# shuklaayush/halo2-plonky2-verifier

Measured on AMD Instinct MI355X. Metric: FRI-verifier witness cells/sec, higher is better.
Workload: dtype u64

## Files before the change

halo2-plonky2-verifier_amd/csrc/coop.h:

```cpp
#pragma once
#include <type_traits>
#include "valbackend.h"
#include "bntab.h"
#include "glptab.h"

namespace h2w {

constexpr int GLP_RECS_FULL = 12 + 48 + 1 + 12 * 14;
constexpr int GLP_RECS_PARTIAL_ROUND = 4 + 1 + 1 + 11 + 1 + 11;
constexpr int GLP_RECS_PARTIAL = 12 + 1 + 121 + N_PARTIAL_ROUNDS * GLP_RECS_PARTIAL_ROUND;
constexpr int GLP_CONST_WORDS = 360 + 12 + 12 + 12 + 22 + 121 + 242 + 242;
constexpr int GLP_RECS = 2 * HALF_N_FULL_ROUNDS * GLP_RECS_FULL + GLP_RECS_PARTIAL;

__device__ __forceinline__ void wave_sync() { asm volatile("s_waitcnt lgkmcnt(0)" ::: "memory"); __builtin_amdgcn_wave_barrier(); }

__shared__ uint64_t s_glp_k[GLP_CONST_WORDS];
__shared__ uint64_t s_glp_a[SPONGE_WIDTH], s_glp_b[SPONGE_WIDTH];
__shared__ uint64_t s_glp_in[CH_BUF];
__shared__ uint64_t s_glp_m[SPONGE_WIDTH * SPONGE_WIDTH];
__shared__ uint64_t s_glp_x[GLP_AUX_WORDS];
typedef __attribute__((address_space(3))) uint64_t lds64_t;
constexpr int KO_ARC = 0, KO_CIRC = 360, KO_DIAG = 372, KO_FIRST = 384, KO_PRC = 396, KO_INIT = 418, KO_WHAT = 539, KO_VS = 781;
static_assert(KO_VS + 242 == GLP_CONST_WORDS, "Goldilocks constant block layout");
template <bool AUX = false> __device__ __forceinline__ void stage_glp_consts(const h2w_poseidon_consts_t *k, int tid, int nthreads) {
    const uint64_t *src = reinterpret_cast<const uint64_t *>(k);
    for (int i = tid; i < GLP_CONST_WORDS; i += nthreads) s_glp_k[i] = g_load_u64(src + i);
    if constexpr (AUX) { const uint64_t *ax = reinterpret_cast<const uint64_t *>(k + 1); for (int i = tid; i < GLP_AUX_WORDS; i += nthreads) s_glp_x[i] = g_load_u64(ax + i); }
    for (int i = tid; i < SPONGE_WIDTH * SPONGE_WIDTH; i += nthreads) {
        const int r = i / SPONGE_WIDTH, j = i % SPONGE_WIDTH; int d = j - r; if (d < 0) d += SPONGE_WIDTH;
        const uint64_t c = g_load_u64(src + KO_CIRC + d);
        s_glp_m[i] = j == r ? gl_reduce128((u128)c + g_load_u64(src + KO_DIAG + r)) : c;
    }
    __syncthreads();
}
inline bool glp_small_mds(const h2w_poseidon_consts_t &k) {
    for (int i = 0; i < SPONGE_WIDTH; i++) if (k.mds_circ[i] >= (1ull << 26) || k.mds_diag[i] >= (1ull << 26)) return false;
    return true;
}

__device__ __forceinline__ uint64_t gl_add_c(uint64_t x, uint64_t y) {
    uint64_t t = x + y;
    if (t < x || t >= GL_P) t -= GL_P;
    return t;
}
__device__ __forceinline__ uint64_t shfl_up64(uint64_t v, int d) { return __shfl_up(v, d, 64); }

__device__ __forceinline__ uint64_t readlane64(uint64_t v, int src) {
    const unsigned lo = (unsigned)__builtin_amdgcn_readlane((int)(unsigned)v, src), hi = (unsigned)__builtin_amdgcn_readlane((int)(unsigned)(v >> 32), src);
    return ((uint64_t)hi << 32) | lo;
}
template <int N> __device__ __forceinline__ uint64_t row_shr64(uint64_t v) {
    const unsigned lo = (unsigned)__builtin_amdgcn_update_dpp(0, (int)(unsigned)v, 0x110 + N, 0xf, 0xf, true);
    const unsigned hi = (unsigned)__builtin_amdgcn_update_dpp(0, (int)(unsigned)(v >> 32), 0x110 + N, 0xf, 0xf, true);
    return ((uint64_t)hi << 32) | lo;
}
}
#include "glperm.h"
namespace h2w {
constexpr int GLP_LIST_WORDS = 1 + SPONGE_WIDTH;

template <bool COLS, bool VALPH = false, int HASH_MODE = -1> struct CoopSinkT : SinkBase {
    static constexpr bool kCoop = true, kDevSponge = VALPH; static constexpr int kHashMode = HASH_MODE;
    rec_t *recs; uint64_t nrec; fr_t *out; uint64_t cell_off; const uint16_t *ncells; int lane; ColPolicy<COLS> cc;
    lds64_t *lk = nullptr, *la = nullptr, *lb = nullptr, *lm = nullptr, *lx = nullptr;
    uint64_t *glp = nullptr; uint32_t glp_slot = 0; bool small_mds = false;
    __device__ __forceinline__ void bind_lds() { lk = (lds64_t *)s_glp_k; la = (lds64_t *)s_glp_a; lb = (lds64_t *)s_glp_b; lm = (lds64_t *)s_glp_m; if constexpr (VALPH) lx = (lds64_t *)s_glp_x; }
    bool emit = true;
    __device__ __forceinline__ void rec(int t, uint64_t a, uint64_t b, uint64_t c, uint64_t d) {
        if (lane == 0 && emit) g_store_rec(recs + nrec, a, b, c, d);
        nrec++; cell_off += ncells[t];
    }
    __device__ __forceinline__ void cell(const fr_t &v) { if (lane == 0 && emit) g_store_fr(out + cc.map(cell_off), v); cell_off++; }
    __device__ __forceinline__ void skip(uint64_t nr, uint64_t nc) { nrec += nr; cell_off += nc; }
    __device__ __forceinline__ bool coop_load_proof(const ValCfg &cfg) { nrec += cfg.load_nrec; cell_off += cfg.load_ncell; return true; }
    uint64_t sx = 0; int sp_in = 0, sp_out = 0; lds64_t *lin = nullptr;
    __device__ __forceinline__ void sponge_init() { sx = 0; sp_in = sp_out = 0; lin = (lds64_t *)s_glp_in; }
    __device__ __forceinline__ bool sponge_observe(uint64_t t) { sp_out = 0; if (sp_in >= CH_BUF) return false; lin[sp_in++] = t; return true; }
    template <class WordFn> __device__ __forceinline__ bool sponge_observe_words(const uint64_t *proof, int n, WordFn word) {
        sp_out = 0; if (sp_in + n > CH_BUF) return false;
        for (int base = 0; base < n; base += 64) { const int i = base + lane; if (i < n) lin[sp_in + i] = g_load_u64(proof + word(i)); }
        sp_in += n; return true;
    }
    template <class WordFn> __device__ __forceinline__ void stage_words(const uint64_t *proof, int at, int n, WordFn word) {
        for (int base = 0; base < n; base += 64) { const int i = base + lane; if (i < n) lin[at + i] = g_load_u64(proof + word(i)); }
    }
    __device__ __forceinline__ uint64_t staged_word(int i) const { return lin[i]; }
    __device__ __forceinline__ bool sponge_observe_cap(const uint64_t *proof, uint64_t w0, int n, int mode, int L) {
        const int per = mode == 0 ? 4 : 5;
        sp_out = 0; if (sp_in + per * n > CH_BUF) return false;
        for (int base = 0; base < n; base += 64) {
            const int j = base + lane;
            if (j < n) {
                fr_t x; for (int i = 0; i < 4; i++) x.l[i] = g_load_u64(proof + w0 + 4ull * j + i);
                if (mode == 0) for (int i = 0; i < 4; i++) lin[sp_in + 4 * j + i] = x.l[i];
                else for (int t = 0; t < 5; t++) lin[sp_in + 5 * j + t] = fr_bits(x, 56 * t, 56);
            }
        }
        sp_in += per * n;
        if (mode == 1) { const int nl = (56 + L - 1) / L, rem = 56 % L; cell_off += (uint64_t)n * (13 + 5ull * ((nl > 1 ? 1 + 3 * (nl - 1) : 0) + (rem ? 4 : 0))); }
        return true;
    }
    __device__ __forceinline__ void sponge_permute() {
        const uint64_t up = row_shr64<1>(sx), w = lane == 0 ? nrec : up;
        uint64_t *at = emit && lane < GLP_LIST_WORDS ? glp + (uint64_t)glp_slot * GLP_LIST_WORDS + lane : nullptr;
        glp_slot++;
        sx = glp_permute_lanes(sx, lk, lm, lx, lane, small_mds, at, w);
        nrec += GLP_RECS;
        cell_off += perm_cell_count();
    }
    uint64_t perm_cells_ = 0;
    __device__ __forceinline__ uint64_t perm_cell_count() {
        if (perm_cells_ == 0) {
            const uint64_t nG = ncells[T_GLOP], nKA = ncells[T_KA_GLOP];
            perm_cells_ = 2 * HALF_N_FULL_ROUNDS * (12 * nKA + 48 * nG + 12 + 12 * (1 + 13 * nKA)) + 12 * nKA + 12 + 121 * nKA + (uint64_t)N_PARTIAL_ROUNDS * (4 * nG + nKA + nKA + 11 * nKA + 12 + 11 * nKA);
        }
        return perm_cells_;
    }
    __device__ __forceinline__ uint64_t sponge_challenge() {
        if (sp_in) {
            for (int off = 0; off < sp_in; off += SPONGE_RATE) {
                const int len = sp_in - off < SPONGE_RATE ? sp_in - off : SPONGE_RATE;
                if ((lane & 15) < len) sx = lin[off + (lane & 15)];
                sponge_permute();
            }
            sp_in = 0; sp_out = SPONGE_RATE;
        } else if (sp_out == 0) { sponge_permute(); sp_out = SPONGE_RATE; }
        return readlane64(sx, --sp_out);
    }

#if defined(H2W_FLATTEN_CHIPS)
    __device__ __forceinline__
#else
    __device__ __noinline__
#endif
    void coop_poseidon_permute(uint64_t *st, const h2w_poseidon_consts_t *) {
        if constexpr (VALPH) {
            uint64_t w = nrec, x = 0;
#pragma unroll
            for (int i = 0; i < SPONGE_WIDTH; i++) { if (lane == i + 1) w = st[i]; if ((lane & 15) == i) x = st[i]; }
            uint64_t *at = emit && lane < GLP_LIST_WORDS ? glp + (uint64_t)glp_slot * GLP_LIST_WORDS + lane : nullptr;
            glp_slot++;
            x = glp_permute_lanes(x, lk, lm, lx, lane, small_mds, at, w);
#pragma unroll
            for (int i = 0; i < SPONGE_WIDTH; i++) st[i] = readlane64(x, i);
            nrec += GLP_RECS;
            cell_off += perm_cell_count();
            return;
        }
        lds64_t *const K = lk, *const s_a = la, *const s_b = lb;
        rec_t *R = recs + nrec;
        const int l = lane, grp13 = lane / 13, idx13 = lane % 13;
        const bool em = emit;
        auto W = [&](int idx, uint64_t A, uint64_t B, uint64_t C) { if (em) g_store_rec(R + idx, A, B, C, 0); };
        if (l < SPONGE_WIDTH) s_a[l] = st[l];
        wave_sync();
        int base = 0, round_ctr = 0;
        auto full_round = [&]() {
            if (l < SPONGE_WIDTH) {
                uint64_t x = s_a[l]; const uint64_t rc = K[KO_ARC + l + SPONGE_WIDTH * round_ctr];
                W(base + l, rc, 1, x); x = gl_add(x, rc);
                const int sb = base + 12 + 4 * l;
                const uint64_t x2 = gl_mul(x, x); W(sb, x, x, 0);
                const uint64_t x4 = gl_mul(x2, x2); W(sb + 1, x2, x2, 0);
                const uint64_t x6 = gl_mul(x4, x2); W(sb + 2, x4, x2, 0);
                const uint64_t x7 = gl_mul(x6, x); W(sb + 3, x6, x, 0);
                s_b[l] = x7;
            }
            wave_sync();
            const int mb = base + 60;
            if (l == 0) W(mb, 0, 0, 0);
            uint64_t rowres = 0;
#pragma unroll
            for (int pass = 0; pass < 3; pass++) {
                const int rr = pass * 4 + grp13;
                uint64_t c = 0, v = 0, x = 0;
                if (l < 52) {
                    if (idx13 < 12) { c = K[KO_CIRC + idx13]; int vi = idx13 + rr; if (vi >= 12) vi -= 12; v = s_b[vi]; }
                    else { c = K[KO_DIAG + rr]; v = s_b[rr]; }
                    x = gl_mul(c, v);
                }
#pragma unroll
                for (int d = 1; d < 16; d <<= 1) { const uint64_t y = shfl_up64(x, d); if (idx13 >= d) x = gl_add_c(x, y); }
                uint64_t prev = shfl_up64(x, 1); if (idx13 == 0) prev = 0;
                if (l < 52) {
                    const int rb = mb + 1 + 14 * rr;
                    if (idx13 == 0) W(rb, 0, 0, 0);
                    W(rb + 1 + idx13, c, v, prev);
                    if (idx13 == 12) rowres = x;
                }
                if (l < 52 && idx13 == 12) s_a[rr] = rowres;
            }
            wave_sync();
            base += GLP_RECS_FULL; round_ctr++;
        };
        for (int i = 0; i < HALF_N_FULL_ROUNDS; i++) full_round();
        if (l < SPONGE_WIDTH) {
            const uint64_t x = s_a[l], c = K[KO_FIRST + l];
            W(base + l, c, 1, x); s_b[l] = gl_add(x, c);
        }
        wave_sync();
        base += 12;
        if (l == 0) { W(base, 0, 0, 0); s_a[0] = s_b[0]; }
        else if (l < SPONGE_WIDTH) {
            uint64_t res = 0;
            for (int r = 1; r < SPONGE_WIDTH; r++) {
                const uint64_t t = K[KO_INIT + (r - 1) * 11 + (l - 1)], v = s_b[r];
                W(base + 1 + (r - 1) * 11 + (l - 1), t, v, res); res = gl_muladd(t, v, res);
            }
            s_a[l] = res;
        }
        wave_sync();
        base += 122;
        for (int r = 0; r < N_PARTIAL_ROUNDS; r++) {
            if (l == 0) {
                const uint64_t x = s_a[0];
                const uint64_t x2 = gl_mul(x, x); W(base, x, x, 0);
                const uint64_t x4 = gl_mul(x2, x2); W(base + 1, x2, x2, 0);
                const uint64_t x6 = gl_mul(x4, x2); W(base + 2, x4, x2, 0);
                const uint64_t x7 = gl_mul(x6, x); W(base + 3, x6, x, 0);
                const uint64_t c = K[KO_PRC + r];
                W(base + 4, c, 1, x7); s_a[0] = gl_add(x7, c);
            }
            wave_sync();
            const uint64_t s0 = s_a[0];
            {
                uint64_t t = 0, v = 0, x = 0;
                if (l == 0) { t = K[KO_CIRC] + K[KO_DIAG]; v = s0; }
                else if (l < SPONGE_WIDTH) { t = K[KO_WHAT + r * 11 + (l - 1)]; v = s_a[l]; }
                if (l < SPONGE_WIDTH) x = gl_mul(t, v);
#pragma unroll
                for (int d = 1; d < 16; d <<= 1) { const uint64_t y = shfl_up64(x, d); if (l >= d) x = gl_add_c(x, y); }
                uint64_t prev = shfl_up64(x, 1); if (l == 0) prev = 0;
                if (l < SPONGE_WIDTH) W(base + 5 + l, t, v, prev);
                if (l == 0) W(base + 17, 0, 0, 0);
                if (l == SPONGE_WIDTH - 1) s_b[0] = x;
                if (l > 0 && l < SPONGE_WIDTH) {
                    const uint64_t tv = K[KO_VS + r * 11 + (l - 1)];
                    W(base + 17 + l, tv, s0, v); s_b[l] = gl_muladd(tv, s0, v);
                }
            }
            wave_sync();
            if (l < SPONGE_WIDTH) s_a[l] = s_b[l];
            wave_sync();
            base += GLP_RECS_PARTIAL_ROUND;
        }
        round_ctr += N_PARTIAL_ROUNDS;
        for (int i = 0; i < HALF_N_FULL_ROUNDS; i++) full_round();
        for (int i = 0; i < SPONGE_WIDTH; i++) st[i] = s_a[i];
        wave_sync();
        const uint64_t nG = ncells[T_GLOP], nKA = ncells[T_KA_GLOP];
        const uint64_t full_cells = 12 * nKA + 48 * nG + 12 + 12 * (1 + 13 * nKA);
        const uint64_t part_cells = 12 * nKA + 12 + 121 * nKA + (uint64_t)N_PARTIAL_ROUNDS * (4 * nG + nKA + nKA + 11 * nKA + 12 + 11 * nKA);
        nrec += GLP_RECS; cell_off += 2 * HALF_N_FULL_ROUNDS * full_cells + part_cells;
    }
};

#ifndef H2W_QUAD_BLOCK
#define H2W_QUAD_BLOCK 256
#endif
constexpr int QUAD_BLOCK = H2W_QUAD_BLOCK;
constexpr int QUAD_WAVES = QUAD_BLOCK / 64;
struct __attribute__((aligned(16))) sq16_t { unsigned long long x, y; };
__shared__ sq16_t s_bn_tab[BK_X * 2];
__shared__ sq16_t s_bn_val[QUAD_WAVES * BN_NSLOT * BN_SLOT_SQ];
__device__ __forceinline__ void stage_bn_consts(const fr_t *tab, int tid, int nthreads) {
    const sq16_t *src = reinterpret_cast<const sq16_t *>(tab);
    for (int i = tid; i < BK_X * 2; i += nthreads) { sq16_t v; v.x = H2W_GLOAD64(&src[i].x); v.y = H2W_GLOAD64(&src[i].y); s_bn_tab[i] = v; }
    __syncthreads();
}
__device__ __forceinline__ fr_t bnk(int which, int idx) {
    const sq16_t a = s_bn_tab[(which * BK_T + idx) * 2], b = s_bn_tab[(which * BK_T + idx) * 2 + 1];
    fr_t r; r.l[0] = a.x; r.l[1] = a.y; r.l[2] = b.x; r.l[3] = b.y; return r;
}
__device__ __forceinline__ fr_t bnkc(int r) {
    const sq16_t a = s_bn_tab[(BK_XC + r) * 2], b = s_bn_tab[(BK_XC + r) * 2 + 1];
    fr_t v; v.l[0] = a.x; v.l[1] = a.y; v.l[2] = b.x; v.l[3] = b.y; return v;
}
__shared__ uint32_t s_bn_tab9[BK9_N * BK9_W];
__device__ __forceinline__ void stage_bn_consts9(const uint32_t *tab9, int tid, int nthreads) {
    const sq16_t *src = reinterpret_cast<const sq16_t *>(tab9); sq16_t *dst = reinterpret_cast<sq16_t *>(s_bn_tab9);
    for (int i = tid; i < BK9_N * BK9_W / 4; i += nthreads) { sq16_t v; v.x = H2W_GLOAD64(&src[i].x); v.y = H2W_GLOAD64(&src[i].y); dst[i] = v; }
    __syncthreads();
}
__device__ __forceinline__ fr9_t bnk9(int idx) {
    const uint4 a = *reinterpret_cast<const uint4 *>(s_bn_tab9 + idx * BK9_W), b = *reinterpret_cast<const uint4 *>(s_bn_tab9 + idx * BK9_W + 4);
    fr9_t v; v.t[0] = a.x; v.t[1] = a.y; v.t[2] = a.z; v.t[3] = a.w; v.t[4] = b.x; v.t[5] = b.y; v.t[6] = b.z; v.t[7] = b.w; v.t[8] = s_bn_tab9[idx * BK9_W + 8];
    return v;
}
template <int CTRL> __device__ __forceinline__ fr_t quad_dpp(const fr_t &v) {
    fr_t r;
#pragma unroll
    for (int i = 0; i < 4; i++) {
        const unsigned lo = (unsigned)v.l[i], hi = (unsigned)(v.l[i] >> 32);
        const unsigned rlo = (unsigned)__builtin_amdgcn_update_dpp(0, (int)lo, CTRL, 0xf, 0xf, false);
        const unsigned rhi = (unsigned)__builtin_amdgcn_update_dpp(0, (int)hi, CTRL, 0xf, 0xf, false);
        r.l[i] = ((unsigned long long)rhi << 32) | rlo;
    }
    return r;
}
template <int J> __device__ __forceinline__ fr_t quad_bcast(const fr_t &v) { return quad_dpp<J * 0x55>(v); }
__device__ __forceinline__ fr_t quad_up1(const fr_t &v) { return quad_dpp<0x90>(v); }
__device__ __forceinline__ fr_t quad_up2(const fr_t &v) { return quad_dpp<0x44>(v); }

template <int CTRL> __device__ __forceinline__ fr9_t quad_dpp9(const fr9_t &v) {
    fr9_t r;
#pragma unroll
    for (int i = 0; i < 9; i++) r.t[i] = (uint32_t)__builtin_amdgcn_update_dpp(0, (int)v.t[i], CTRL, 0xf, 0xf, false);
    return r;
}
template <int J> __device__ __forceinline__ fr9_t quad_bcast9(const fr9_t &v) { return quad_dpp9<J * 0x55>(v); }
__device__ __forceinline__ fr9_t fr9_sel(bool c, const fr9_t &a, const fr9_t &b) {
    fr9_t r;
#pragma unroll
    for (int i = 0; i < 9; i++) r.t[i] = c ? a.t[i] : b.t[i];
    return r;
}
__device__ __forceinline__ fr9_t fr9_add_if(bool c, const fr9_t &a, const fr9_t &b) {
    fr9_t r;
#pragma unroll
    for (int i = 0; i < 9; i++) r.t[i] = a.t[i] + (c ? b.t[i] : 0u);
    return r;
}
__device__ __forceinline__ fr_t fr_sel(bool c, const fr_t &a, const fr_t &b) {
    fr_t r;
#pragma unroll
    for (int i = 0; i < 4; i++) r.l[i] = c ? a.l[i] : b.l[i];
    return r;
}
struct BnSrc { int kind, idx; };
constexpr BnSrc bV(int s) { return BnSrc{0, s}; }
constexpr BnSrc bK(int i) { return BnSrc{1, i}; }
constexpr BnSrc bA(int o) { return BnSrc{2, o}; }
constexpr BnSrc bB(int o) { return BnSrc{3, o}; }
constexpr BnSrc bn_map_exp5(int c) {
    const int l = c / 12, i = c % 12;
    return (i == 0 || i == 4 || i == 8) ? bK(BK_ZERO) : (i == 1 || i == 2 || i == 10) ? bV(l) : (i == 3 || i == 5 || i == 6) ? bV(4 + l) : (i == 7 || i == 9) ? bV(8 + l) : bV(12 + l);
}
constexpr BnSrc bn_map_ark(int c) {
    const int l = c / 5, i = c % 5;
    return (i == 0 || i == 2) ? bA(l) : i == 1 ? bV(l) : i == 3 ? bK(BK_ONE) : bV(4 + l);
}
constexpr BnSrc bn_map_mix(int c) {
    const int l = c / 16, j = (c % 16) / 4, i = c % 4;
    return i == 0 ? (j == 0 ? bK(BK_ZERO) : bV(4 + 4 * l + j - 1)) : i == 1 ? bA(4 * j + l) : i == 2 ? bV(j) : bV(4 + 4 * l + j);
}
constexpr BnSrc bn_map_consts(int c) { return bA(c); }
constexpr BnSrc bn_map_zero(int) { return bK(BK_ZERO); }
constexpr BnSrc bn_map_partial(int c) {
    if (c < 12) return (c == 0 || c == 4 || c == 8) ? bK(BK_ZERO) : (c == 1 || c == 2 || c == 10) ? bV(0) : (c == 3 || c == 5 || c == 6) ? bV(4) : (c == 7 || c == 9) ? bV(5) : bV(6);
    if (c < 17) return (c == 12 || c == 14) ? bB(0) : c == 13 ? bV(6) : c == 15 ? bK(BK_ONE) : bV(7);
    if (c < 37) { const int j = (c - 17) / 5, i = (c - 17) % 5; return (i == 0 || i == 2) ? bA(j) : i == 1 ? (j == 0 ? bK(BK_ZERO) : bV(8 + j - 1)) : i == 3 ? (j == 0 ? bV(7) : bV(j)) : bV(8 + j); }
    const int k = 1 + (c - 37) / 5, i = (c - 37) % 5;
    return (i == 0 || i == 2) ? bA(4 + k - 1) : i == 1 ? bV(k) : i == 3 ? bV(7) : bV(12 + k - 1);
}

enum { QUAD_VALUES = 1, QUAD_EMIT = 2, QUAD_FUSED = 3 };
constexpr int QUAD_VERDICT = 4;
template <bool COLS, int MODE> struct QuadSinkT : SinkBase {
    static constexpr bool kBnUnits = true; static constexpr int kHashMode = 1;
    rec_t *recs; uint64_t nrec; fr_t *out; uint64_t cell_off; const uint16_t *ncells; int l4; ColPolicy<COLS> cc;
    fr_t *ustate;
    fr_t *sbx;
    int unit_local = 0;
    int my_w = 0, last_w = 0;
    bool act = true;
    __device__ __forceinline__ void set_window(int w, int n_units) { my_w = w; last_w = n_units > 0 ? n_units - 1 : 0; unit_local = 0; act = w == 0; }
    __device__ __forceinline__ void rec(int t, uint64_t a, uint64_t b, uint64_t c, uint64_t d) {
        if (MODE != QUAD_VALUES && l4 == 0 && act) g_store_rec(recs + nrec, a, b, c, d);
        nrec++; cell_off += ncells[t];
    }
    __device__ __forceinline__ void cell(const fr_t &v) { if (MODE != QUAD_VALUES && l4 == 0 && act) g_store_fr(out + cc.map(cell_off), v); cell_off++; }
    __device__ __forceinline__ void skip(uint64_t nr, uint64_t nc) { nrec += nr; cell_off += nc; }
    struct Em {
        sq16_t *val;
        const sq16_t *tabh;
        unsigned long long gdst;
        uint64_t cell0;
        int l;
        ColPolicy<COLS> cc;
    };
    static __device__ __forceinline__ void put(const Em &e, int slot, const fr_t &v) {
        sq16_t *q = e.val + slot * BN_SLOT_SQ; q[0] = sq16_t{v.l[0], v.l[1]}; q[1] = sq16_t{v.l[2], v.l[3]};
    }
    static __device__ __forceinline__ void put_if(const Em &e, bool on, int slot, const fr_t &v) { if (on) put(e, slot, v); }
    template <class MapFn> static __device__ __forceinline__ const sq16_t *src_ptr(const Em &e, MapFn map, int c, const sq16_t *baseA, const sq16_t *baseB) {
        const BnSrc s = map(c);
        return s.kind == 0 ? e.val + s.idx * BN_SLOT_SQ + (e.l & 1) : s.kind == 1 ? e.tabh + s.idx * 2 : s.kind == 2 ? baseA + s.idx * 2 : baseB + s.idx * 2;
    }
    template <int N, class MapFn> __device__ __forceinline__ void flush_layer(Em &e, MapFn map, const sq16_t *baseA, const sq16_t *baseB) {
        constexpr int NP = (N + 1) / 2;
        const bool hiq = e.l >= 2;
        if constexpr (COLS) {
            if (e.cc.hi - e.cell0 < (uint64_t)N || e.cell0 < e.cc.lo) { e = flush_layer_cols<N>(e, map, baseA, baseB); return; }
        }
#pragma unroll
        for (int k0 = 0; k0 < NP; k0 += 4) {
            sq16_t t[4];
#pragma unroll
            for (int u = 0; u < 4; u++) {
                const int k = k0 + u;
                if (k < NP) {
                    const sq16_t *pa = src_ptr(e, map, 2 * k, baseA, baseB), *pb = (2 * k + 1 < N) ? src_ptr(e, map, 2 * k + 1, baseA, baseB) : pa;
                    t[u] = *(hiq ? pb : pa);
                }
            }
#pragma unroll
            for (int u = 0; u < 4; u++) {
                const int k = k0 + u;
                if (k < NP) {
                    unsigned long long *g = reinterpret_cast<unsigned long long *>(e.gdst + (unsigned long long)k * 64);
                    if (2 * k + 1 < N || !hiq) { H2W_GSTORE64(g, t[u].x); H2W_GSTORE64(g + 1, t[u].y); }
                }
            }
        }
        e.cell0 += (uint64_t)N; e.gdst += (unsigned long long)N * 32;
    }
    template <int K0, int K1, int N, class MapFn> static __device__ __forceinline__ void part_load(const Em &e, MapFn map, const sq16_t *baseA, const sq16_t *baseB, sq16_t *t) {
        const bool hiq = e.l >= 2;
#pragma unroll
        for (int k = K0; k < K1; k++) {
            const sq16_t *pa = src_ptr(e, map, 2 * k, baseA, baseB), *pb = (2 * k + 1 < N) ? src_ptr(e, map, 2 * k + 1, baseA, baseB) : pa;
            t[k - K0] = *(hiq ? pb : pa);
        }
    }
    template <int K0, int K1, int N> static __device__ __forceinline__ void part_store(const Em &e, const sq16_t *t) {
        const bool hiq = e.l >= 2;
#pragma unroll
        for (int k = K0; k < K1; k++) {
            unsigned long long *g = reinterpret_cast<unsigned long long *>(e.gdst + (unsigned long long)k * 64);
            if (2 * k + 1 < N || !hiq) { H2W_GSTORE64(g, t[k - K0].x); H2W_GSTORE64(g + 1, t[k - K0].y); }
        }
    }
    typedef __attribute__((address_space(3))) const sq16_t lds_sq16;
    struct Wide { int off0, off1, kind0, kind1; bool has1; int lane; unsigned long long gq; };
    static __device__ __forceinline__ void wide_desc(int pc, int &off, int &kind) {
        const int c = pc >> 1; const BnSrc sd = bn_map_partial(c < 52 ? c : 51);
        kind = sd.kind; off = (sd.kind == 0 ? sd.idx * BN_SLOT_SQ : sd.idx * 2) + (pc & 1);
    }
    static __device__ __forceinline__ Wide wide_init(const Em &e) {
        Wide w; w.lane = threadIdx.x & 63; w.has1 = w.lane < 2 * 52 - 64;
        wide_desc(w.lane, w.off0, w.kind0); wide_desc(w.has1 ? 64 + w.lane : 0, w.off1, w.kind1);
        w.gq = e.gdst - (unsigned long long)e.l * 16;
        return w;
    }
    template <int Q0, int Q1> static __device__ __forceinline__ void wide_load(const Wide &w, lds_sq16 *valw, lds_sq16 *tab, lds_sq16 *baseA, lds_sq16 *baseB, sq16_t *t0, sq16_t *t1) {
        lds_sq16 *b0 = (w.kind0 == 0 ? valw : w.kind0 == 1 ? tab : w.kind0 == 2 ? baseA : baseB) + w.off0;
        lds_sq16 *b1 = (w.kind1 == 0 ? valw : w.kind1 == 1 ? tab : w.kind1 == 2 ? baseA : baseB) + w.off1;
        const int q0 = w.kind0 == 0 ? 2 : 0, q1 = w.kind1 == 0 ? 2 : 0;
#pragma unroll
        for (int q = Q0; q < Q1; q++) { t0[q - Q0].x = b0[q * q0].x; t0[q - Q0].y = b0[q * q0].y; t1[q - Q0].x = b1[q * q1].x; t1[q - Q0].y = b1[q * q1].y; }
    }
    template <int Q0, int Q1> static __device__ __forceinline__ void wide_store(const Wide &w, const sq16_t *t0, const sq16_t *t1) {
#pragma unroll
        for (int q = Q0; q < Q1; q++) {
            const unsigned long long gb = readlane64(w.gq, 4 * q) + (unsigned long long)w.lane * 16;
            unsigned long long *g = reinterpret_cast<unsigned long long *>(gb);
            H2W_GSTORE64(g, t0[q - Q0].x); H2W_GSTORE64(g + 1, t0[q - Q0].y);
            if (w.has1) { H2W_GSTORE64(g + 128, t1[q - Q0].x); H2W_GSTORE64(g + 129, t1[q - Q0].y); }
        }
    }
    template <int N, class MapFn> __device__ __noinline__ Em flush_layer_cols(Em e, MapFn map, const sq16_t *baseA, const sq16_t *baseB) {
        if constexpr (COLS) {
            const bool hiq = e.l >= 2;
            for (int k = 0; k < (N + 1) / 2; k++) {
                const int c = 2 * k + (hiq ? 1 : 0);
                if (c < N) {
                    const sq16_t *pa = src_ptr_rt(e, map, 2 * k, baseA, baseB), *pb = (2 * k + 1 < N) ? src_ptr_rt(e, map, 2 * k + 1, baseA, baseB) : pa;
                    const sq16_t t = *(hiq ? pb : pa);
                    const uint64_t a = e.cc.map(e.cell0 + (uint64_t)c);
                    unsigned long long *g = reinterpret_cast<unsigned long long *>(reinterpret_cast<unsigned long long>(out + a) + (unsigned long long)(e.l & 1) * 16);
                    H2W_GSTORE64(g, t.x); H2W_GSTORE64(g + 1, t.y);
                }
            }
            e.cell0 += (uint64_t)N;
            e.gdst = reinterpret_cast<unsigned long long>(out + e.cc.map(e.cell0)) + (unsigned long long)e.l * 16;
        }
        return e;
    }
    template <class MapFn> static __device__ __forceinline__ const sq16_t *src_ptr_rt(const Em &e, MapFn map, int c, const sq16_t *baseA, const sq16_t *baseB) {
        const BnSrc s = map(c);
        return s.kind == 0 ? e.val + s.idx * BN_SLOT_SQ + (e.l & 1) : s.kind == 1 ? e.tabh + s.idx * 2 : s.kind == 2 ? baseA + s.idx * 2 : baseB + s.idx * 2;
    }
    __device__ __forceinline__ bool level_skip(fr_t &node, bool &zc_ref) {
        if constexpr (MODE != QUAD_EMIT) return false;
        else {
            const int k = unit_local;
            if (k == my_w) return false;
            if (k + 1 == my_w) node = g_load_fr(ustate + (uint64_t)k * 4);
            if (!zc_ref) { cell_off += 1; zc_ref = true; }
            cell_off += 2 * 8 + 4 + BN_PERM_CELLS;
            unit_local = k + 1;
            const int cur = unit_local < last_w ? unit_local : last_w;
            act = cur == my_w;
            return true;
        }
    }
    __device__ __forceinline__ bool tail_skip() const { return MODE == QUAD_VALUES || (MODE == QUAD_EMIT && !act); }
    __device__ __forceinline__ bool bn_emit_inline(fr_t *st, const ValCfg &cfg, bool &zc_ref) {
        if constexpr (MODE == QUAD_VALUES || MODE == QUAD_VERDICT) { bn_values(st, cfg); unit_local++; return true; }
        else if constexpr (MODE == QUAD_FUSED) { bn_emit_cells<false>(st, cfg, zc_ref); return true; }
        else {
            const int k = unit_local++;
            if (k == my_w) bn_emit_cells<true>(st, cfg, zc_ref);
            else {
                if (k + 1 == my_w) {
                    const fr_t *u = ustate + (uint64_t)k * 4;
#pragma unroll
                    for (int i = 0; i < 4; i++) st[i] = g_load_fr(u + i);
                }
                if (!zc_ref) { cell_off += 1; zc_ref = true; }
                cell_off += BN_PERM_CELLS;
            }
            const int cur = unit_local < last_w ? unit_local : last_w;
            act = cur == my_w;
            return true;
        }
    }
    __device__ __noinline__ void bn_values(fr_t *st, const ValCfg &cfg) {
        const int l = l4, lm = l > 0 ? l - 1 : 0; const uint32_t ninv = (uint32_t)cfg.P.ninv & ((1u << 29) - 1);
        fr_t *const sbu = sbx + (uint64_t)unit_local * (BN_PARTIAL_ROUNDS * 3);
        fr9_t S = fr9_mont(fr9_from(fr_sel(l < 2, fr_sel(l == 0, st[0], st[1]), fr_sel(l == 2, st[2], st[3]))), fr9_from(cfg.P.r2), ninv);
        auto sbox = [&]() { const fr9_t X2 = fr9_mont(S, S, ninv), X4 = fr9_mont(X2, X2, ninv); S = fr9_mont(X4, S, ninv); };
        auto mix = [&](int mb) {
            const fr9_t s0 = quad_bcast9<0>(S), s1 = quad_bcast9<1>(S), s2 = quad_bcast9<2>(S), s3 = quad_bcast9<3>(S);
            fr9_t acc = fr9_mont(s0, bnk9(mb + l), ninv);
            acc = fr9_add(fr9_mont(s1, bnk9(mb + 4 + l), ninv), acc);
            acc = fr9_add(fr9_mont(s2, bnk9(mb + 8 + l), ninv), acc);
            S = fr9_norm(fr9_add(fr9_mont(s3, bnk9(mb + 12 + l), ninv), acc));
        };
        S = fr9_norm(fr9_add(S, bnk9(BK_C + l)));
#pragma unroll 1
        for (int half = 0; half < 2; half++) {
            if (half == 1) {
                fr9_t s0p; for (int i = 0; i < 9; i++) s0p.t[i] = 0;
                struct RoundK { fr9_t kp, k2, k1, kc, kx; };
                auto round_k = [&](int r) {
                    const int ix = BK_S + (BN_WIDTH * 2 - 1) * r, ic = BK_C + (BN_FULL_ROUNDS / 2 + 1) * BN_WIDTH + r;
                    RoundK k; k.kp = bnk9(ix - (BN_WIDTH * 2 - 1) + BN_WIDTH + lm);
                    k.k2 = bnk9(ix + (l == 1 ? 0 : l)); k.k1 = bnk9(ix + 1); k.kc = bnk9(ic); k.kx = bnk9(BK9_X + r);
                    return k;
                };
                RoundK kc_ = round_k(0);
#pragma unroll 2
                for (int r = 0; r < BN_PARTIAL_ROUNDS; r++) {
                    const RoundK kn = round_k(r + 1 < BN_PARTIAL_ROUNDS ? r + 1 : r);
                    fr_t *const sb = sbu + (uint64_t)r * 3;
                    const fr9_t s0b = quad_bcast9<0>(S);
                    const fr9_t A_ = fr9_mont(fr9_sel(l == 0, S, s0p), fr9_sel(l == 0, S, kc_.kp), ninv);
                    if constexpr (MODE != QUAD_VERDICT) { if (l == 0) g_store_fr(sb, fr9_pack(A_)); }
                    const fr9_t X2b = quad_bcast9<0>(A_);
                    S = fr9_add_if(l > 0, S, A_);
                    const fr9_t B_ = fr9_mont(fr9_sel(l == 0, X2b, fr9_sel(l == 1, s0b, S)), fr9_sel(l == 0, X2b, kc_.k2), ninv);
                    if constexpr (MODE != QUAD_VERDICT) { if (l == 0) g_store_fr(sb + 1, fr9_pack(B_)); }
                    const fr9_t X4b = quad_bcast9<0>(B_), XAb = quad_bcast9<1>(B_);
                    const fr9_t C_ = fr9_mont(fr9_sel(l == 1, S, X4b), fr9_sel(l == 0, XAb, fr9_sel(l == 1, kc_.k1, s0b)), ninv);
                    if constexpr (MODE != QUAD_VERDICT) { if (l == 2) g_store_fr(sb + 2, fr9_pack(C_)); }
                    s0p = fr9_add(quad_bcast9<2>(C_), kc_.kc);
                    fr9_t incl = fr9_add_if(l == 0, fr9_sel(l < 2, C_, B_), kc_.kx);
                    incl = fr9_add(incl, quad_dpp9<0xB1>(incl));
                    incl = fr9_add(incl, quad_dpp9<0x4E>(incl));
                    S = fr9_norm(fr9_sel(l == 0, incl, S));
                    kc_ = kn;
                }
                {
                    const fr9_t U = fr9_mont(s0p, bnk9(BK_S + (BN_WIDTH * 2 - 1) * (BN_PARTIAL_ROUNDS - 1) + BN_WIDTH + lm), ninv);
                    S = fr9_norm(fr9_add_if(l > 0, S, U));
                }
            }
#pragma unroll 1
            for (int r = 0; r < BN_FULL_ROUNDS / 2; r++) {
                const bool last = r == BN_FULL_ROUNDS / 2 - 1;
                sbox();
                if (!(half == 1 && last)) S = fr9_add(S, bnk9(BK_C + (half == 0 ? (r + 1) * BN_WIDTH : (BN_FULL_ROUNDS / 2 + 1) * BN_WIDTH + BN_PARTIAL_ROUNDS + r * BN_WIDTH) + l));
                mix(half == 0 && last ? BK_P : BK_M);
            }
        }
        fr9_t one9; for (int i = 0; i < 9; i++) one9.t[i] = i == 0 ? 1u : 0u;
        fr_t s = fr9_pack(fr9_mont(S, one9, ninv));
        if (fr_geq_mod(s)) s = fr_sub_mod_raw(s);
        if constexpr (MODE != QUAD_VERDICT) g_store_fr(ustate + (uint64_t)unit_local * 4 + l, s);
        st[0] = quad_bcast<0>(s); st[1] = quad_bcast<1>(s); st[2] = quad_bcast<2>(s); st[3] = quad_bcast<3>(s);
    }
    template <bool PRE> __device__ __noinline__ void bn_emit_cells(fr_t *st, const ValCfg &cfg, bool &zc_ref) {
        bool zc = zc_ref;
        const int l = l4; const uint64_t ninv = cfg.P.ninv; const fr_t r2 = cfg.P.r2;
        Em e; e.l = l;
        const int val_off = ((threadIdx.x >> 6) * BN_NSLOT * BN_SLOT_SQ) + ((threadIdx.x & 63) >> 2) * 2;
        e.val = s_bn_val + val_off;
        e.tabh = s_bn_tab + (l & 1);
        e.cell0 = cell_off;
        e.cc = cc;
        e.gdst = reinterpret_cast<unsigned long long>(out + e.cc.map(cell_off)) + (unsigned long long)l * 16;
        fr_t s = fr_sel(l < 2, fr_sel(l == 0, st[0], st[1]), fr_sel(l == 2, st[2], st[3]));
        auto exp5_all = [&]() {
            const fr_t X = fr_mont_mul(s, r2, ninv);
            const fr_t x2 = fr_mont_mul(s, X, ninv), X2 = fr_mont_mul(X, X, ninv);
            const fr_t x4 = fr_mont_mul(x2, X2, ninv), x5 = fr_mont_mul(x4, X, ninv);
            put(e, l, s); put(e, 4 + l, x2); put(e, 8 + l, x4); put(e, 12 + l, x5);
            flush_layer<48>(e, bn_map_exp5, e.tabh, e.tabh);
            s = x5;
        };
        auto ark = [&](int it) {
            const fr_t ns = fr_add(s, bnk(0, BK_C + it + l));
            put(e, l, s); put(e, 4 + l, ns);
            flush_layer<20>(e, bn_map_ark, e.tabh + (BK_C + it) * 2, e.tabh);
            s = ns;
        };
        auto mix = [&](int which) {
            if (!zc) { flush_layer<1>(e, bn_map_zero, e.tabh, e.tabh); zc = true; }
            const int mb = which ? BK_P : BK_M;
            put(e, l, s);
            fr_t acc = fr_zero();
#pragma unroll 1
            for (int j = 0; j < 4; j++) {
                const sq16_t a0 = e.val[j * BN_SLOT_SQ], a1 = e.val[j * BN_SLOT_SQ + 1];
                fr_t sj; sj.l[0] = a0.x; sj.l[1] = a0.y; sj.l[2] = a1.x; sj.l[3] = a1.y;
                acc = fr_add(fr_mont_mul(sj, bnk(1, mb + 4 * j + l), ninv), acc);
                put(e, 4 + 4 * l + j, acc);
            }
            flush_layer<64>(e, bn_map_mix, e.tabh + mb * 2, e.tabh);
            s = acc;
        };
        ark(0);
#pragma unroll 1
        for (int half = 0; half < 2; half++) {
            if (half == 1) {
                if constexpr (PRE) {
                    const fr_t *sb = sbx + (uint64_t)my_w * (BN_PARTIAL_ROUNDS * 3) + (l < 3 ? l : 2);
                    Wide wd = wide_init(e);
                    lds_sq16 *const valw = (lds_sq16 *)s_bn_val + (threadIdx.x >> 6) * BN_NSLOT * BN_SLOT_SQ;
                    auto round = [&](int r, const fr_t &qv, auto pend_tag) {
                        const int ix = BK_S + (BN_WIDTH * 2 - 1) * r, lm = l > 0 ? l - 1 : 0, ic = BK_C + (BN_FULL_ROUNDS / 2 + 1) * BN_WIDTH + r;
                        constexpr bool pend = !COLS && decltype(pend_tag)::value;
                        lds_sq16 *const tab = (lds_sq16 *)s_bn_tab, *const wA = tab + (ix - (BN_WIDTH * 2 - 1)) * 2, *const wB = tab + (ic - 1) * 2;
                        sq16_t t0[6], t1[6], u0[5], u1[5], v0[5], v1[5];
                        const fr_t x2 = quad_bcast<0>(qv), x4 = quad_bcast<1>(qv), x5 = quad_bcast<2>(qv);
                        const fr_t s0n = fr_add(x5, bnk(0, ic));
                        const fr_t ksxm = bnk(1, ix + l);
                        if (pend) wide_load<0, 6>(wd, valw, tab, wA, wB, t0, t1);
                        const fr_t P_ = fr_mont_mul(fr_sel(l == 0, s0n, s), ksxm, ninv);
                        if (pend) { wide_store<0, 6>(wd, t0, t1); wide_load<6, 11>(wd, valw, tab, wA, wB, u0, u1); }
                        const fr_t Q_ = fr_mont_mul(s0n, bnk(1, ix + BN_WIDTH + lm), ninv);
                        if (pend) { wide_store<6, 11>(wd, u0, u1); wide_load<11, 16>(wd, valw, tab, wA, wB, v0, v1); }
                        fr_t incl = P_;
                        { const fr_t t = quad_up1(incl); if (l >= 1) incl = fr_add(incl, t); }
                        { const fr_t t = quad_up2(incl); if (l >= 2) incl = fr_add(incl, t); }
                        const fr_t nv = fr_add(Q_, s);
                        if (pend) { wide_store<11, 16>(wd, v0, v1); e.cell0 += 52; e.gdst += 52ull * 32; wd.gq += 52ull * 32; }
                        put(e, l, s);
                        put_if(e, l == 0, 4, x2); put_if(e, l == 0, 5, x4); put_if(e, l == 0, 6, x5); put_if(e, l == 0, 7, s0n);
                        put(e, 8 + l, incl);
                        put_if(e, l > 0, 12 + lm, nv);
                        const fr_t ns0 = quad_bcast<3>(incl);
                        s = fr_sel(l > 0, nv, ns0);
                        if (COLS || r == BN_PARTIAL_ROUNDS - 1) flush_layer<52>(e, bn_map_partial, e.tabh + ix * 2, e.tabh + ic * 2);
                    };
                    static_assert(BN_PARTIAL_ROUNDS % 2 == 0, "rounds are walked in pairs");
                    fr_t qc0 = g_load_fr(sb + 3), qc1 = g_load_fr(sb + 6);
                    { const fr_t q = g_load_fr(sb); round(0, q, std::false_type()); }
                    asm volatile("" :: "v"(qc0.l[0]), "v"(qc0.l[2]), "v"(qc1.l[0]), "v"(qc1.l[2]));
#pragma unroll 1
                    for (int r = 1; r < BN_PARTIAL_ROUNDS - 1; r += 2) {
                        const int rn = r + 2 < BN_PARTIAL_ROUNDS - 1 ? r + 2 : r;
                        const fr_t qn0 = g_load_fr(sb + 3 * rn), qn1 = g_load_fr(sb + 3 * (rn + 1));
                        round(r, qc0, std::true_type()); round(r + 1, qc1, std::true_type());
                        qc0 = qn0; qc1 = qn1;
                    }
                    { const fr_t q = g_load_fr(sb + 3 * (BN_PARTIAL_ROUNDS - 1)); round(BN_PARTIAL_ROUNDS - 1, q, std::true_type()); }
                } else {
                    fr_t s0p = fr_zero();
                    const int lm = l > 0 ? l - 1 : 0;
#pragma unroll 1
                    for (int r = 0; r < BN_PARTIAL_ROUNDS; r++) {
                        const int ix = BK_S + (BN_WIDTH * 2 - 1) * r, ic = BK_C + (BN_FULL_ROUNDS / 2 + 1) * BN_WIDTH + r;
                        const bool pend = !COLS && r > 0;
                        const sq16_t *pA = e.tabh + (ix - (BN_WIDTH * 2 - 1)) * 2, *pB = e.tabh + (ic - 1) * 2;
                        sq16_t t0[7], t1[7], t2[6], t3[6];
                        if (pend) part_load<0, 7, 52>(e, bn_map_partial, pA, pB, t0);
                        const fr_t A_ = fr_mont_mul(fr_sel(l == 0, s, s0p), fr_sel(l == 0, r2, bnk(1, ix - (BN_WIDTH * 2 - 1) + BN_WIDTH + lm)), ninv);
                        if (r > 0) { const fr_t nv = fr_add(A_, s); put_if(e, l > 0, 12 + lm, nv); s = fr_sel(l > 0, nv, s); }
                        if (COLS && r > 0) flush_layer<52>(e, bn_map_partial, pA, pB);
                        if (pend) { part_store<0, 7, 52>(e, t0); part_load<7, 14, 52>(e, bn_map_partial, pA, pB, t1); }
                        const fr_t Xb = quad_bcast<0>(A_), s0b = quad_bcast<0>(s);
                        const fr_t B_ = fr_mont_mul(fr_sel(l == 1, s0b, fr_sel(l == 3, s, Xb)), fr_sel(l < 2, Xb, bnk(1, ix + (l == 2 ? 0 : l))), ninv);
                        if (pend) { part_store<7, 14, 52>(e, t1); part_load<14, 20, 52>(e, bn_map_partial, pA, pB, t2); }
                        const fr_t x2b = quad_bcast<1>(B_), XSb = quad_bcast<2>(B_);
                        const fr_t C_ = fr_mont_mul(fr_sel(l == 0, x2b, s), fr_sel(l == 0, B_, bnk(1, ix + l)), ninv);
                        if (pend) { part_store<14, 20, 52>(e, t2); part_load<20, 26, 52>(e, bn_map_partial, pA, pB, t3); }
                        const fr_t D_ = fr_mont_mul(quad_bcast<0>(C_), fr_sel(l == 0, XSb, Xb), ninv);
                        if (pend) { part_store<20, 26, 52>(e, t3); e.cell0 += 52; e.gdst += 52ull * 32; }
                        const fr_t s0n = fr_add(quad_bcast<1>(D_), bnk(0, ic));
                        put(e, l, s);
                        put_if(e, l == 1, 4, B_); put_if(e, l == 0, 5, C_); put_if(e, l == 1, 6, D_); put_if(e, l == 0, 7, s0n);
                        fr_t incl = fr_sel(l == 0, fr_add(D_, bnkc(r)), fr_sel(l == 3, B_, C_));
                        { const fr_t t = quad_up1(incl); if (l >= 1) incl = fr_add(incl, t); }
                        { const fr_t t = quad_up2(incl); if (l >= 2) incl = fr_add(incl, t); }
                        put(e, 8 + l, incl);
                        s0p = s0n;
                        s = fr_sel(l == 0, quad_bcast<3>(incl), s);
                    }
                    {
                        const fr_t U = fr_mont_mul(s0p, bnk(1, BK_S + (BN_WIDTH * 2 - 1) * (BN_PARTIAL_ROUNDS - 1) + BN_WIDTH + lm), ninv);
                        const fr_t nv = fr_add(U, s); put_if(e, l > 0, 12 + lm, nv); s = fr_sel(l > 0, nv, s);
                        const int ixl = BK_S + (BN_WIDTH * 2 - 1) * (BN_PARTIAL_ROUNDS - 1), icl = BK_C + (BN_FULL_ROUNDS / 2 + 1) * BN_WIDTH + BN_PARTIAL_ROUNDS - 1;
                        flush_layer<52>(e, bn_map_partial, e.tabh + ixl * 2, e.tabh + icl * 2);
                    }
                }
            }
            flush_layer<32>(e, bn_map_consts, e.tabh + BK_M * 2, e.tabh);
#pragma unroll 1
            for (int r = 0; r < BN_FULL_ROUNDS / 2; r++) {
                const bool last = r == BN_FULL_ROUNDS / 2 - 1;
                { int vo = val_off, ll = l; asm volatile("" : "+v"(vo), "+v"(ll)); e.val = s_bn_val + vo; e.tabh = s_bn_tab + (ll & 1); e.l = ll; }
                exp5_all();
                if (!(half == 1 && last)) ark(half == 0 ? (r + 1) * BN_WIDTH : (BN_FULL_ROUNDS / 2 + 1) * BN_WIDTH + BN_PARTIAL_ROUNDS + r * BN_WIDTH);
                mix(half == 0 && last ? 1 : 0);
            }
        }
        st[0] = quad_bcast<0>(s); st[1] = quad_bcast<1>(s); st[2] = quad_bcast<2>(s); st[3] = quad_bcast<3>(s);
        cell_off = e.cell0; zc_ref = zc; cc = e.cc;
    }
};

}
```

Before: 184.9 billion.

## Align partial-round witness stores to cache lines and defer layer tails

Reworks how each 52-cell partial Poseidon layer is written to global memory. Each lane's 16-byte store pieces are shifted so they line up with 128-byte lines, and the last pieces of a layer are held back and written together with the next layer. To keep the deferred sources valid, the slot-7 state is double-buffered between slots 7 and 15, and new source kinds are added for the previous round's values. The aim is fewer partial-line global writes, at the cost of more complex address and selection logic and a risk of subtle write-ordering bugs.

Result: slower. 182.9 billion (-1.1%).

```diff
diff --git a/halo2-plonky2-verifier_amd/csrc/chainvisits.h b/halo2-plonky2-verifier_amd/csrc/chainvisits.h
--- /dev/null
+++ b/halo2-plonky2-verifier_amd/csrc/chainvisits.h
@@ -0,0 +1,13 @@
+#pragma once
+namespace h2w {
+enum { CV_ARK = 0, CV_CONSTS = 1, CV_EXP5 = 2, CV_MIX = 3, CV_PARTIAL = 4, CV_ZERO = 5 };
+constexpr int CV_LINE_B = 128, CV_CELL_B = 32, CV_PIECE_B = 16;
+constexpr int cv_layer_cells(int kind) { return kind == CV_ARK ? 20 : kind == CV_CONSTS ? 32 : kind == CV_EXP5 ? 48 : kind == CV_MIX ? 64 : kind == CV_PARTIAL ? 52 : 1; }
+constexpr int cv_line_off(unsigned long long first_cell_byte_addr) { return (int)((first_cell_byte_addr % CV_LINE_B) / CV_CELL_B); }
+constexpr bool cv_defers(int kind, int next_kind) { return (kind == CV_PARTIAL || kind == CV_MIX) && next_kind == CV_PARTIAL; }
+constexpr int cv_first_deferred(int n_cells, int o) { return 2 * n_cells - 2 * o; }
+constexpr bool cv_piece_deferred(int n_cells, int o, int piece) { return piece >= cv_first_deferred(n_cells, o); }
+constexpr int cv_quad_piece(int step, int lane) { return 4 * step + lane; }
+constexpr bool cv_shifted(int o) { return (o & 1) != 0; }
+constexpr int cv_quad_piece_shifted(int step, int lane) { return 4 * step + lane - 2; }
+}
diff --git a/halo2-plonky2-verifier_amd/csrc/coop.h b/halo2-plonky2-verifier_amd/csrc/coop.h
--- a/halo2-plonky2-verifier_amd/csrc/coop.h
+++ b/halo2-plonky2-verifier_amd/csrc/coop.h
@@ -2,6 +2,7 @@
 #include <type_traits>
 #include "valbackend.h"
 #include "bntab.h"
+#include "chainvisits.h"
 #include "glptab.h"
 
 namespace h2w {
@@ -354,6 +355,9 @@
     return (i == 0 || i == 2) ? bA(4 + k - 1) : i == 1 ? bV(k) : i == 3 ? bV(7) : bV(12 + k - 1);
 }
 
+constexpr BnSrc bn_map_partial_s7(int c) { const BnSrc s = bn_map_partial(c); return s.kind == 0 && s.idx == 7 ? BnSrc{4, 0} : s; }
+constexpr BnSrc bn_map_partial_tail(int c) { return c == 49 ? BnSrc{4, 2} : c == 50 ? BnSrc{4, 1} : c == 51 ? bV(3) : bn_map_partial(c); }
+
 enum { QUAD_VALUES = 1, QUAD_EMIT = 2, QUAD_FUSED = 3 };
 constexpr int QUAD_VERDICT = 4;
 template <bool COLS, int MODE> struct QuadSinkT : SinkBase {
@@ -377,6 +381,8 @@
         unsigned long long gdst;
         uint64_t cell0;
         int l;
+        const sq16_t *s7;
+        const sq16_t *s7o, *t49;
         ColPolicy<COLS> cc;
     };
     static __device__ __forceinline__ void put(const Em &e, int slot, const fr_t &v) {
@@ -385,9 +391,9 @@
     static __device__ __forceinline__ void put_if(const Em &e, bool on, int slot, const fr_t &v) { if (on) put(e, slot, v); }
     template <class MapFn> static __device__ __forceinline__ const sq16_t *src_ptr(const Em &e, MapFn map, int c, const sq16_t *baseA, const sq16_t *baseB) {
         const BnSrc s = map(c);
-        return s.kind == 0 ? e.val + s.idx * BN_SLOT_SQ + (e.l & 1) : s.kind == 1 ? e.tabh + s.idx * 2 : s.kind == 2 ? baseA + s.idx * 2 : baseB + s.idx * 2;
-    }
-    template <int N, class MapFn> __device__ __forceinline__ void flush_layer(Em &e, MapFn map, const sq16_t *baseA, const sq16_t *baseB) {
+        return s.kind == 4 ? (s.idx == 2 ? e.t49 : (s.idx ? e.s7o : e.s7) + (e.l & 1)) : s.kind == 0 ? e.val + s.idx * BN_SLOT_SQ + (e.l & 1) : s.kind == 1 ? e.tabh + s.idx * 2 : s.kind == 2 ? baseA + s.idx * 2 : baseB + s.idx * 2;
+    }
+    template <int N, class MapFn> __device__ __forceinline__ void flush_layer(Em &e, MapFn map, const sq16_t *baseA, const sq16_t *baseB, bool keep24 = true, bool keep25 = true) {
         constexpr int NP = (N + 1) / 2;
         const bool hiq = e.l >= 2;
         if constexpr (COLS) {
@@ -409,7 +415,7 @@
                 const int k = k0 + u;
                 if (k < NP) {
                     unsigned long long *g = reinterpret_cast<unsigned long long *>(e.gdst + (unsigned long long)k * 64);
-                    if (2 * k + 1 < N || !hiq) { H2W_GSTORE64(g, t[u].x); H2W_GSTORE64(g + 1, t[u].y); }
+                    if ((2 * k + 1 < N || !hiq) && (k != NP - 2 || keep24) && (k != NP - 1 || keep25)) { H2W_GSTORE64(g, t[u].x); H2W_GSTORE64(g + 1, t[u].y); }
                 }
             }
         }
@@ -430,6 +436,42 @@
             unsigned long long *g = reinterpret_cast<unsigned long long *>(e.gdst + (unsigned long long)k * 64);
             if (2 * k + 1 < N || !hiq) { H2W_GSTORE64(g, t[k - K0].x); H2W_GSTORE64(g + 1, t[k - K0].y); }
         }
+    }
+    struct Tail { bool odd, ge2, d24, d25; };
+    static __device__ __forceinline__ Tail tail_init(const Em &e) {
+        if constexpr (COLS) return Tail{false, false, false, false};
+        else {
+            const int o = cv_line_off(e.gdst - (unsigned long long)e.l * 16);
+            return Tail{cv_shifted(o), cv_first_deferred(52, o) <= 2 * 52 - 4, cv_piece_deferred(52, o, cv_quad_piece(24, e.l)), cv_piece_deferred(52, o, cv_quad_piece(25, e.l))};
+        }
+    }
+    template <int K0, int K1> static __device__ __forceinline__ void line_load(const Em &e, const sq16_t *baseA, const sq16_t *baseB, sq16_t *t, Tail tl) {
+        const bool hiq = e.l >= 2, same = tl.odd == hiq;
+#pragma unroll
+        for (int k = K0; k < K1; k++) {
+            const sq16_t *c0 = src_ptr(e, bn_map_partial_s7, 2 * k, baseA, baseB), *cp = src_ptr(e, bn_map_partial_s7, 2 * k + 1, baseA, baseB);
+            const sq16_t *cm = k > 0 ? src_ptr(e, bn_map_partial_s7, 2 * k - 1, baseA, baseB) : src_ptr(e, bn_map_partial_tail, 51, baseA, baseB);
+            const sq16_t *p = same ? c0 : (hiq ? cp : cm);
+            if (k == 25) {
+                const sq16_t *q0 = src_ptr(e, bn_map_partial_tail, 50, baseA, baseB), *qp = src_ptr(e, bn_map_partial_tail, 51, baseA, baseB), *qm = src_ptr(e, bn_map_partial_tail, 49, baseA, baseB);
+                p = tl.ge2 ? (same ? q0 : (hiq ? qp : qm)) : p;
+            }
+            t[k - K0] = *p;
+        }
+    }
+    template <int K0, int K1> static __device__ __forceinline__ void line_store(const Em &e, const sq16_t *t, Tail tl) {
+#pragma unroll
+        for (int k = K0; k < K1; k++) {
+            unsigned long long *g = reinterpret_cast<unsigned long long *>(e.gdst + (unsigned long long)k * 64 - (k == 25 && tl.ge2 ? 52ull * 32 : 0ull));
+            H2W_GSTORE64(g, t[k - K0].x); H2W_GSTORE64(g + 1, t[k - K0].y);
+        }
+    }
+    static __device__ __forceinline__ void tail_flush(const Em &e, Tail tl, const sq16_t *baseA, const sq16_t *baseB) {
+        const bool hiq = e.l >= 2;
+        const sq16_t t24 = *src_ptr(e, bn_map_partial_tail, 49, baseA, baseB);
+        const sq16_t t25 = *(hiq ? src_ptr(e, bn_map_partial_tail, 51, baseA, baseB) : src_ptr(e, bn_map_partial_tail, 50, baseA, baseB));
+        if (tl.d24) { unsigned long long *g = reinterpret_cast<unsigned long long *>(e.gdst - 2ull * 64); H2W_GSTORE64(g, t24.x); H2W_GSTORE64(g + 1, t24.y); }
+        if (tl.d25) { unsigned long long *g = reinterpret_cast<unsigned long long *>(e.gdst - 1ull * 64); H2W_GSTORE64(g, t25.x); H2W_GSTORE64(g + 1, t25.y); }
     }
     typedef __attribute__((address_space(3))) const sq16_t lds_sq16;
     struct Wide { int off0, off1, kind0, kind1; bool has1; int lane; unsigned long long gq; };
@@ -479,7 +521,7 @@
     }
     template <class MapFn> static __device__ __forceinline__ const sq16_t *src_ptr_rt(const Em &e, MapFn map, int c, const sq16_t *baseA, const sq16_t *baseB) {
         const BnSrc s = map(c);
-        return s.kind == 0 ? e.val + s.idx * BN_SLOT_SQ + (e.l & 1) : s.kind == 1 ? e.tabh + s.idx * 2 : s.kind == 2 ? baseA + s.idx * 2 : baseB + s.idx * 2;
+        return s.kind == 4 ? (s.idx == 2 ? e.t49 : (s.idx ? e.s7o : e.s7) + (e.l & 1)) : s.kind == 0 ? e.val + s.idx * BN_SLOT_SQ + (e.l & 1) : s.kind == 1 ? e.tabh + s.idx * 2 : s.kind == 2 ? baseA + s.idx * 2 : baseB + s.idx * 2;
     }
     __device__ __forceinline__ bool level_skip(fr_t &node, bool &zc_ref) {
         if constexpr (MODE != QUAD_EMIT) return false;
@@ -588,6 +630,7 @@
         const int val_off = ((threadIdx.x >> 6) * BN_NSLOT * BN_SLOT_SQ) + ((threadIdx.x & 63) >> 2) * 2;
         e.val = s_bn_val + val_off;
         e.tabh = s_bn_tab + (l & 1);
+        e.s7 = e.s7o = e.val + 7 * BN_SLOT_SQ; e.t49 = e.tabh;
         e.cell0 = cell_off;
         e.cc = cc;
         e.gdst = reinterpret_cast<unsigned long long>(out + e.cc.map(cell_off)) + (unsigned long long)l * 16;
@@ -618,7 +661,12 @@
                 acc = fr_add(fr_mont_mul(sj, bnk(1, mb + 4 * j + l), ninv), acc);
                 put(e, 4 + 4 * l + j, acc);
             }
-            flush_layer<64>(e, bn_map_mix, e.tabh + mb * 2, e.tabh);
+            if (COLS || PRE) flush_layer<64>(e, bn_map_mix, e.tabh + mb * 2, e.tabh);
+            else {
+                const Tail tl = tail_init(e);
+                flush_layer<64>(e, bn_map_mix, e.tabh + mb * 2, e.tabh, !(which && tl.d24), !(which && tl.d25));
+                if (which) e.val[15 * BN_SLOT_SQ + (l & 1)] = e.val[3 * BN_SLOT_SQ + (l & 1)];
+            }
             s = acc;
         };
         ark(0);
@@ -670,28 +718,34 @@
                 } else {
                     fr_t s0p = fr_zero();
                     const int lm = l > 0 ? l - 1 : 0;
+                    const Tail tl = tail_init(e);
+                    if (tl.odd) e.gdst -= 32;
 #pragma unroll 1
                     for (int r = 0; r < BN_PARTIAL_ROUNDS; r++) {
                         const int ix = BK_S + (BN_WIDTH * 2 - 1) * r, ic = BK_C + (BN_FULL_ROUNDS / 2 + 1) * BN_WIDTH + r;
                         const bool pend = !COLS && r > 0;
                         const sq16_t *pA = e.tabh + (ix - (BN_WIDTH * 2 - 1)) * 2, *pB = e.tabh + (ic - 1) * 2;
-                        sq16_t t0[7], t1[7], t2[6], t3[6];
-                        if (pend) part_load<0, 7, 52>(e, bn_map_partial, pA, pB, t0);
+                        sq16_t *const s7r = e.val + (COLS || (r & 1) == 0 ? 7 : 15) * BN_SLOT_SQ;
+                        e.s7 = COLS || (r & 1) ? e.val + 7 * BN_SLOT_SQ : e.val + 15 * BN_SLOT_SQ;
+                        e.s7o = s7r; e.t49 = r == 1 ? e.tabh + (BK_P + 15) * 2 : e.tabh + (ix - 2 * (BN_WIDTH * 2 - 1) + 6) * 2;
+                        sq16_t t0[7], t1[7], t2[7], t3[5];
+                        if (pend) line_load<0, 7>(e, pA, pB, t0, tl);
                         const fr_t A_ = fr_mont_mul(fr_sel(l == 0, s, s0p), fr_sel(l == 0, r2, bnk(1, ix - (BN_WIDTH * 2 - 1) + BN_WIDTH + lm)), ninv);
                         if (r > 0) { const fr_t nv = fr_add(A_, s); put_if(e, l > 0, 12 + lm, nv); s = fr_sel(l > 0, nv, s); }
                         if (COLS && r > 0) flush_layer<52>(e, bn_map_partial, pA, pB);
-                        if (pend) { part_store<0, 7, 52>(e, t0); part_load<7, 14, 52>(e, bn_map_partial, pA, pB, t1); }
+                        if (pend) { line_store<0, 7>(e, t0, tl); line_load<7, 13>(e, pA, pB, t1, tl); line_load<25, 26>(e, pA, pB, t1 + 6, tl); }
                         const fr_t Xb = quad_bcast<0>(A_), s0b = quad_bcast<0>(s);
                         const fr_t B_ = fr_mont_mul(fr_sel(l == 1, s0b, fr_sel(l == 3, s, Xb)), fr_sel(l < 2, Xb, bnk(1, ix + (l == 2 ? 0 : l))), ninv);
-                        if (pend) { part_store<7, 14, 52>(e, t1); part_load<14, 20, 52>(e, bn_map_partial, pA, pB, t2); }
+                        if (pend) { line_store<7, 13>(e, t1, tl); line_store<25, 26>(e, t1 + 6, tl); line_load<13, 20>(e, pA, pB, t2, tl); }
                         const fr_t x2b = quad_bcast<1>(B_), XSb = quad_bcast<2>(B_);
                         const fr_t C_ = fr_mont_mul(fr_sel(l == 0, x2b, s), fr_sel(l == 0, B_, bnk(1, ix + l)), ninv);
-                        if (pend) { part_store<14, 20, 52>(e, t2); part_load<20, 26, 52>(e, bn_map_partial, pA, pB, t3); }
+                        if (pend) { line_store<13, 20>(e, t2, tl); line_load<20, 25>(e, pA, pB, t3, tl); }
                         const fr_t D_ = fr_mont_mul(quad_bcast<0>(C_), fr_sel(l == 0, XSb, Xb), ninv);
-                        if (pend) { part_store<20, 26, 52>(e, t3); e.cell0 += 52; e.gdst += 52ull * 32; }
+                        if (pend) { line_store<20, 25>(e, t3, tl); e.cell0 += 52; e.gdst += 52ull * 32; }
                         const fr_t s0n = fr_add(quad_bcast<1>(D_), bnk(0, ic));
                         put(e, l, s);
-                        put_if(e, l == 1, 4, B_); put_if(e, l == 0, 5, C_); put_if(e, l == 1, 6, D_); put_if(e, l == 0, 7, s0n);
+                        put_if(e, l == 1, 4, B_); put_if(e, l == 0, 5, C_); put_if(e, l == 1, 6, D_);
+                        if (l == 0) { s7r[0] = sq16_t{s0n.l[0], s0n.l[1]}; s7r[1] = sq16_t{s0n.l[2], s0n.l[3]}; }
                         fr_t incl = fr_sel(l == 0, fr_add(D_, bnkc(r)), fr_sel(l == 3, B_, C_));
                         { const fr_t t = quad_up1(incl); if (l >= 1) incl = fr_add(incl, t); }
                         { const fr_t t = quad_up2(incl); if (l >= 2) incl = fr_add(incl, t); }
@@ -702,8 +756,12 @@
                     {
                         const fr_t U = fr_mont_mul(s0p, bnk(1, BK_S + (BN_WIDTH * 2 - 1) * (BN_PARTIAL_ROUNDS - 1) + BN_WIDTH + lm), ninv);
                         const fr_t nv = fr_add(U, s); put_if(e, l > 0, 12 + lm, nv); s = fr_sel(l > 0, nv, s);
+                        if (tl.odd) e.gdst += 32;
                         const int ixl = BK_S + (BN_WIDTH * 2 - 1) * (BN_PARTIAL_ROUNDS - 1), icl = BK_C + (BN_FULL_ROUNDS / 2 + 1) * BN_WIDTH + BN_PARTIAL_ROUNDS - 1;
-                        flush_layer<52>(e, bn_map_partial, e.tabh + ixl * 2, e.tabh + icl * 2);
+                        e.s7o = e.val + (COLS || ((BN_PARTIAL_ROUNDS - 1) & 1) ? 7 : 15) * BN_SLOT_SQ; e.s7 = e.val + (COLS || ((BN_PARTIAL_ROUNDS - 1) & 1) == 0 ? 7 : 15) * BN_SLOT_SQ;
+                        e.t49 = e.tabh + (ixl - (BN_WIDTH * 2 - 1) + 6) * 2;
+                        if constexpr (!COLS) { static_assert(BN_PARTIAL_ROUNDS >= 2, "a partial layer keeps its tail back for the partial layer after it"); tail_flush(e, tl, e.tabh + ixl * 2, e.tabh + icl * 2); }
+                        flush_layer<52>(e, bn_map_partial_s7, e.tabh + ixl * 2, e.tabh + icl * 2);
                     }
                 }
             }
```
